# mapillary/OpenSfM

Hardware: AMD Instinct MI355X
Metric: image-pairs matched/sec (+ BA LM-iters/sec, 5k cams / 500k pts) (higher is better)
Workload: dtype i8 (exact int32 accumulate) + f64 RANSAC

## Files before the change

### opensfm_amd/csrc/ba.hip

```cpp
#ifdef OSFM_HIPEMU
#include <cassert>
#endif
#include <chrono>
#include <cmath>
#include <cstdio>
#include <cstring>
#include <numeric>
#include <vector>

#include <rocprim/rocprim.hpp>

#include "ba_math.h"
#include "osfm_internal.h"

using namespace osfm_ba;

namespace {

constexpr int kCoopObs = 256;

typedef double osfm_v2d __attribute__((ext_vector_type(2)));
__device__ __forceinline__ void st2(double *p, double a, double b) {
  osfm_v2d v;
  v.x = a;
// ... 99 lines not shown
        rho1 = a / r;
      } else {
        rho = s;
        rho1 = 1.0;
      }
      break;
    case OSFM_LOSS_CAUCHY: {
      const double sum = 1.0 + s / b;
      rho = b * log(sum);
      rho1 = 1.0 / sum;
    } break;
    default:
      rho = s;
      rho1 = 1.0;
  }
}

template <int NV, int MAXT, int N>
__device__ __forceinline__ void block_sum(double *v, double (&lds)[N]) {
  static_assert(MAXT % 64 == 0 && MAXT <= 1024, "MAXT: the kernel's launch bound, whole wavefronts");
  static_assert(N >= NV * (MAXT / 64), "block_sum: lds is shorter than NV doubles for every wavefront the launch bound allows");
#ifdef OSFM_HIPEMU
  assert((int)blockDim.x <= MAXT);
#endif
#pragma unroll
  for (int k = 0; k < NV; k++)
#pragma unroll
    for (int m = 32; m >= 1; m >>= 1) v[k] += __shfl_xor(v[k], m);
  const int lane = threadIdx.x & 63, w = threadIdx.x >> 6;
  const int nw = (blockDim.x + 63) >> 6;
  if (nw == 1) return;
  if (lane == 0)
#pragma unroll
    for (int k = 0; k < NV; k++) lds[w * NV + k] = v[k];
  __syncthreads();
  if (threadIdx.x == 0)
#pragma unroll
    for (int k = 0; k < NV; k++) {
      double s = lds[k];
      for (int w2 = 1; w2 < nw; w2++) s += lds[w2 * NV + k];
      v[k] = s;
    }
}

template <int NV, int W, int N>
__device__ __forceinline__ void shot_sum(double (&v)[NV], double (&lds)[N] ) {
  static_assert(W == 1 || N >= W * NV, "shot_sum: lds is shorter than NV doubles per wavefront");
#ifdef OSFM_HIPEMU
  assert((int)blockDim.x == 64 * W);
#endif
#pragma unroll
  for (int i = 0; i < NV; i++)
#pragma unroll
    for (int m = 32; m >= 1; m >>= 1) v[i] += __shfl_xor(v[i], m);
  if (W == 1) return;
  const int lane = threadIdx.x & 63, w = threadIdx.x >> 6;
  if (lane == 0)
#pragma unroll
    for (int i = 0; i < NV; i++) lds[w * NV + i] = v[i];
  __syncthreads();
  if (threadIdx.x == 0)
#pragma unroll
    for (int i = 0; i < NV; i++) {
      double t = lds[i];
#pragma unroll
      for (int q = 1; q < W; q++) t += lds[q * NV + i];
      v[i] = t;
    }
}
constexpr int kShotWavesSmall = 4;
constexpr int kShotWavesBelow = 1024;

__device__ __forceinline__ long xcd_contiguous(long b, long n) {
  const long q = n >> 3, r = n & 7;
  const long xcd = b & 7, within = b >> 3;
  return (xcd < r ? xcd * (q + 1) : r * (q + 1) + (xcd - r) * q) + within;
}

struct GenDev {
  int NRr;
  int KW;
  int NB;
  int NV, NRC;
  int oJp, oJc, oJb, ncomp;
  const int *view_inst, *view_rc, *view_cam;
  const int *view_col;
  const long *view_off;
  const int *inst_view0;
  const int *o_view, *sm_view;
  const unsigned char *o_kind, *sm_kind;
  double *cam, *cam_n;
  const double *cam_prior, *cam_sigma;
  double *rc, *rc_n;
  const double *rc_prior, *rc_sigma;
  double *bias, *bias_n;
  double *rcR;
  const unsigned char *rc_useful;
  const int *cam_col, *rc_col, *bias_col;
  const unsigned char *col_slot;
  double *vpart;
  double *yv;
  double *PI, *Bpri, *Cpri;
  double *gpri;
  double *bdot;
  const double *gps, *gps_sigma;
  const int *inst_bias_cam;
  const double *up, *up_sigma;
  const double *pan, *pan_sigma, *tilt, *tilt_sigma, *roll, *roll_sigma;
  const double *pt_prior, *pt_prior_sigma;
  const unsigned char *pt_prior_alt;
};

struct Dev {
  int S, P, NC;
  long M;
  int nred, cam0;
  double *cams, *poses, *pts, *cams_n, *poses_n, *pts_n;
  const double *cam_prior, *cam_sigma, *gps, *gps_sigma;
  const double *up, *up_sigma;
  double *up_r, *up_J;
  double *prior_rot;
  const uint8_t *cam_fixed, *shot_fixed, *point_fixed;
  const int *shot_camera;
  const int *cam_model;
  const double *cam_ext;
  const int *o_shot, *o_point;
  const double *o_x, *o_y, *o_sigma;
  const long *pt_off;
  const int *wg_pt;
  int nwg;
  const long *shot_off;
  const int *shot_obs;
  double *shotR;
  double *Epm;
  double *Jpm;
  double *sm_wt;
  const int *sm_shot, *sm_point;
  const double *sm_x, *sm_y, *sm_sigma;
  double *w;
  double *g_pt, *Hpp, *Hhat, *sc_pt, *D_pt, *d_pt;
  double *g_red, *diag_red, *prior_diag, *sc_red, *D_red;
  double *Hcc;
  double *Binv;
  double *part;
  double *camred;
  int bw;
  double *band;
  const unsigned char *bslot;
  double *dinv;
  const int *bp_pts;
  const int *bp_o0, *bp_last;
  const unsigned char *bp_pos;
  const int *bp_off;
  int bpNT, bpR, bpPC;
  double *bp_part;
  int cs, ncl, ncd;
  double *cD;
  double *cW, *cWt;
  double *cLi, *cLit;
  double *bD, *bE, *bG, *bH;
  double *bD2, *bGt, *bHt;
  double *bx;
  int wNB, wWb;
  double *wA, *wL, *wLt, *wDinv, *wx;
  int qcs, qm, qN;
  double *qD;
  double *qE[2];
  double *qX;
  double *qXt;
  double *qx, *qy;
  int qT;
  double *qP, *qR, *qRn, *qC;
  double *zc;
  double *y;
  double *x, *r, *z, *p, *Ap, *b;
  double *scal;
  double *partial;
  double *partial2;
  double *dotp;
  double *rrp;
  int gen;
  GenDev g;
};

#define JA(o, c) d.Jpm[(long)(c) * d.M + (o)]
constexpr int kRowComps = 17;
constexpr int R_JP = 2, R_JR = 8, R_U = 14, R_V = 15, R_WT = 16;

__device__ __forceinline__ void row_jk(const Dev &d, long o, int s, double (&jk)[6]) {
  const int ci = d.shot_camera[s];
  const double u = JA(o, R_U), v = JA(o, R_V), wt = JA(o, R_WT), sg = d.o_sigma[o];
  const double *cam = d.cams + 3 * ci;
  const double k1 = cam[0], k2 = cam[1], f = cam[2];
  const bool other = d.cam_model && d.cam_model[ci] >= 2;
  double J[6];
  jk_entries(1.0 / sg, k1, k2, f, u, v, J);
#pragma unroll
  for (int i = 0; i < 6; i++) jk[i] = other ? 0.0 : wt * J[i];
}

__global__ void shot_rot_kernel(Dev d, const double *poses) {
  const int s = blockIdx.x * blockDim.x + threadIdx.x;
  if (s >= d.S) return;
  rot_and_derivs(poses + 6 * s, d.shotR + 36 * (long)s, d.shotR + 36 * (long)s + 9);
}

struct ShotFrame {
  int model;
  const double *cam, *pose, *R;
};
__device__ __forceinline__ ShotFrame shot_frame(const Dev &d, int s) {
  const int ci = d.shot_camera[s];
  ShotFrame f;
  f.model = d.cam_model ? d.cam_model[ci] : 0;
  f.cam = f.model >= 2 ? d.cam_ext + 16 * ci : d.cams + 3 * ci;
  f.pose = d.poses + 6 * (long)s;
  f.R = d.shotR + 36 * (long)s;
  return f;
}
__device__ __forceinline__ void sm_row(const Dev &d, const ShotFrame &f, long k, double wt, double (&r)[2], double (&Jp)[6], double (&Jc)[12], double (&Jk)[6]) {
  const int p = d.sm_point[k];
  project_obs<true>(f.model, d.pts + 3 * (long)p, f.pose, f.R, f.R + 9, f.cam, d.sm_x[k], d.sm_y[k], 1.0 / d.sm_sigma[k], r, Jp, Jc, Jk);
  r[0] *= wt;
  r[1] *= wt;
#pragma unroll
  for (int i = 0; i < 6; i++) Jp[i] *= wt;
#pragma unroll
  for (int i = 0; i < 12; i++) Jc[i] *= wt;
#pragma unroll
  for (int i = 0; i < 6; i++) Jk[i] *= wt;
}

template <bool JAC>
__global__ void __launch_bounds__(kCoopObs) eval_kernel(Dev d, const double *cams, const double *poses, const double *pts, int loss, double a) {
  __shared__ double c[JAC ? 9 : 1][kCoopObs];
  __shared__ double lds[8];
  const int tid = threadIdx.x;
  const int p0 = d.wg_pt[blockIdx.x], p1 = d.wg_pt[blockIdx.x + 1];
  const long o0 = d.pt_off[p0], o1 = d.pt_off[p1];
  double acc[2] = {0.0, 0.0};
  auto compute = [&](long o, double (&row)[kRowComps]) {
    const int s = d.o_shot[o], p = d.o_point[o];
    const double *R = d.shotR + 36 * (long)s;
    double r[2], Jp[6], Jc[12], Jk[6], uv[2];
    const double sg = d.o_sigma[o];
    const int cmodel = d.cam_model ? d.cam_model[d.shot_camera[s]] : 0;
    project_obs<JAC>(cmodel, pts + 3 * (long)p, poses + 6 * (long)s, R, R + 9, cmodel >= 2 ? d.cam_ext + 16 * d.shot_camera[s] : cams + 3 * d.shot_camera[s], d.o_x[o],
                     d.o_y[o], 1.0 / sg, r, Jp, Jc, Jk, uv);
    const double sq = r[0] * r[0] + r[1] * r[1];
    double rho, rho1;
    loss_eval(loss, a, sq, rho, rho1);
    acc[0] += 0.5 * rho;
    acc[1] += sq * sg * sg;
    if (JAC) {
      const double wt = sqrt(rho1);
      row[0] = wt * r[0];
      row[1] = wt * r[1];
#pragma unroll
      for (int i = 0; i < 6; i++) row[R_JP + i] = wt * Jp[i];
#pragma unroll
      for (int i = 0; i < 2; i++)
#pragma unroll
        for (int k = 0; k < 3; k++) row[R_JR + 3 * i + k] = wt * Jc[6 * i + k];
      row[R_U] = uv[0];
      row[R_V] = uv[1];
      row[R_WT] = wt;
    }
  };
  auto products = [&](const double (&row)[kRowComps], double (&v)[9]) {
    const double r0 = row[0], r1 = row[1];
    const double *jp = row + R_JP;
#pragma unroll
    for (int j = 0; j < 3; j++) v[j] = jp[j] * r0 + jp[3 + j] * r1;
    v[3] = jp[0] * jp[0] + jp[3] * jp[3];
    v[4] = jp[0] * jp[1] + jp[3] * jp[4];
    v[5] = jp[0] * jp[2] + jp[3] * jp[5];
    v[6] = jp[1] * jp[1] + jp[4] * jp[4];
    v[7] = jp[1] * jp[2] + jp[4] * jp[5];
    v[8] = jp[2] * jp[2] + jp[5] * jp[5];
  };
  auto store = [&](long o, const double (&row)[kRowComps]) {
#pragma unroll
    for (int i = 0; i < kRowComps; i++) __builtin_nontemporal_store(row[i], &JA(o, i));
    if (d.Epm) {
      const double *jp = row + R_JP;
      double2 *dst = reinterpret_cast<double2 *>(d.Epm + 18 * o);
#pragma unroll
      for (int i = 0; i < 6; i += 2) {
        const double a0 = i < 3 ? row[R_JR + i] : -jp[i - 3], b0 = i < 3 ? row[R_JR + 3 + i] : -jp[3 + i - 3];
        const double a1 = i + 1 < 3 ? row[R_JR + i + 1] : -jp[i + 1 - 3], b1 = i + 1 < 3 ? row[R_JR + 3 + i + 1] : -jp[3 + i + 1 - 3];
        double e[6];
#pragma unroll
        for (int j = 0; j < 3; j++) {
          e[j] = a0 * jp[j] + b0 * jp[3 + j];
          e[3 + j] = a1 * jp[j] + b1 * jp[3 + j];
        }
        st2(reinterpret_cast<double *>(dst + 3 * (i / 2)), e[0], e[1]);
        st2(reinterpret_cast<double *>(dst + 3 * (i / 2) + 1), e[2], e[3]);
        st2(reinterpret_cast<double *>(dst + 3 * (i / 2) + 2), e[4], e[5]);
      }
    }
  };
  if (o1 - o0 <= kCoopObs) {
    const bool on = tid < o1 - o0;
    double row[kRowComps];
    if (on) {
      compute(o0 + tid, row);
// ... 448 lines not shown

__device__ __forceinline__ void jred_jp(const Dev &d, long k, double E[6][3]) {
  const double2 *src = reinterpret_cast<const double2 *>(d.Epm + 18 * (long)d.shot_obs[k]);
#pragma unroll
  for (int q = 0; q < 9; q++) {
    const double2 v = src[q];
    E[(2 * q) / 3][(2 * q) % 3] = v.x;
    E[(2 * q + 1) / 3][(2 * q + 1) % 3] = v.y;
  }
}
__global__ void __launch_bounds__(TPB) band_assemble_kernel(Dev d, double radius, int copies, int dk_lo, int ndk) {
  extern __shared__ __attribute__((aligned(16))) double acc[];
  const int s = (int)xcd_contiguous(blockIdx.x, gridDim.x), nb = ndk * 36;
  const int copy = threadIdx.x & (copies - 1);
  for (int t = threadIdx.x; t < nb * copies; t += TPB) acc[t] = 0.0;
  __syncthreads();
  for (long k = d.shot_off[s] + threadIdx.x; k < d.shot_off[s + 1]; k += TPB) {
    const int p = d.sm_point[k];
    const double *Hh = d.Hhat + 6 * (long)p;
    const double h[9] = {Hh[0], Hh[1], Hh[2], Hh[1], Hh[3], Hh[4], Hh[2], Hh[4], Hh[5]};
    double Ea[6][3], EH[6][3];
    jred_jp(d, k, Ea);
#pragma unroll
    for (int i = 0; i < 6; i++)
#pragma unroll
      for (int j = 0; j < 3; j++) EH[i][j] = Ea[i][0] * h[j] + Ea[i][1] * h[3 + j] + Ea[i][2] * h[6 + j];
    for (long o2 = d.pt_off[p]; o2 < d.pt_off[p + 1]; o2++) {
      const int dk = s - d.o_shot[o2] - dk_lo;
      if (dk < 0 || dk >= ndk) continue;
      double Eb[6][3];
      {
        const double2 *src = reinterpret_cast<const double2 *>(d.Epm + 18 * o2);
#pragma unroll
        for (int q = 0; q < 9; q++) {
          const double2 v = src[q];
          Eb[(2 * q) / 3][(2 * q) % 3] = v.x;
          Eb[(2 * q + 1) / 3][(2 * q + 1) % 3] = v.y;
        }
      }
#pragma unroll
      for (int i = 0; i < 6; i++)
#pragma unroll
        for (int j = 0; j < 6; j++)
          atomicAdd(&acc[(dk * 36 + i * 6 + j) * copies + copy], EH[i][0] * Eb[j][0] + EH[i][1] * Eb[j][1] + EH[i][2] * Eb[j][2]);
    }
  }
  __syncthreads();
  for (int t = threadIdx.x; t < nb; t += TPB) {
    const int dk = dk_lo + t / 36, ij = t % 36, i = ij / 6, j = ij % 6;
    const int s2 = s - dk;
    double val = 0.0;
    if (s2 >= 0) {
      double sum = 0.0;
      for (int c = 0; c < copies; c++) sum += acc[t * copies + c];
      val = -sum;
      if (dk == 0) {
        const int hi = i > j ? i : j, lo = i > j ? j : i;
        val += d.Hcc[21 * (long)s + hi * (hi + 1) / 2 + lo];
        if (i == j) val += d.prior_diag[6 * s + i];
      }
      val *= d.sc_red[6 * s + i] * d.sc_red[6 * s2 + j];
      if (dk == 0 && i == j) val += d.D_red[6 * s + i] / radius;
    }
    d.band[((long)s * (d.bw + 1) + dk) * 36 + ij] = val;
  }
}

__global__ void __launch_bounds__(TPB) band_slots_kernel(Dev d, unsigned char *table, int *max_slots) {
  extern __shared__ int bs_present[];
  const int s = blockIdx.x, R1 = d.bw + 1;
  for (int t = threadIdx.x; t < R1; t += TPB) bs_present[t] = 0;
  __syncthreads();
  for (long k = d.shot_off[s] + threadIdx.x; k < d.shot_off[s + 1]; k += TPB) {
    const int p = d.sm_point[k];
    for (long o2 = d.pt_off[p]; o2 < d.pt_off[p + 1]; o2++) {
      const int dk = s - d.o_shot[o2];
      if (dk >= 0 && dk <= d.bw) bs_present[dk] = 1;
    }
  }
  __syncthreads();
  if (threadIdx.x == 0) {
    int n = 0;
    for (int t = 0; t < R1; t++) {
      const bool on = bs_present[t] != 0 || t == 0;
      table[(long)s * R1 + t] = on ? (unsigned char)(n < 255 ? n : 255) : (unsigned char)255;
      n += on ? 1 : 0;
    }
    atomicMax(max_slots, n);
  }
}
__global__ void __launch_bounds__(TPB) band_assemble_compact_kernel(Dev d, double radius, int copies, int nslots) {
  extern __shared__ __attribute__((aligned(16))) double acc[];
  const int s = (int)xcd_contiguous(blockIdx.x, gridDim.x), R1 = d.bw + 1;
  unsigned char *slot = reinterpret_cast<unsigned char *>(acc + (long)nslots * 36 * copies);
  const int copy = threadIdx.x & (copies - 1);
  for (int t = threadIdx.x; t < nslots * 36 * copies; t += TPB) acc[t] = 0.0;
  for (int t = threadIdx.x; t < R1; t += TPB) slot[t] = d.bslot[(long)s * R1 + t];
  __syncthreads();
  for (long k = d.shot_off[s] + threadIdx.x; k < d.shot_off[s + 1]; k += TPB) {
    const int p = d.sm_point[k];
    const double *Hh = d.Hhat + 6 * (long)p;
    const double h[9] = {Hh[0], Hh[1], Hh[2], Hh[1], Hh[3], Hh[4], Hh[2], Hh[4], Hh[5]};
    double Ea[6][3], EH[6][3];
    jred_jp(d, k, Ea);
#pragma unroll
    for (int i = 0; i < 6; i++)
#pragma unroll
      for (int j = 0; j < 3; j++) EH[i][j] = Ea[i][0] * h[j] + Ea[i][1] * h[3 + j] + Ea[i][2] * h[6 + j];
    for (long o2 = d.pt_off[p]; o2 < d.pt_off[p + 1]; o2++) {
      const int dk = s - d.o_shot[o2];
      if (dk < 0 || dk > d.bw) continue;
      const int sl = slot[dk];
      double Eb[6][3];
      {
        const double2 *src = reinterpret_cast<const double2 *>(d.Epm + 18 * o2);
#pragma unroll
        for (int q = 0; q < 9; q++) {
          const double2 v = src[q];
          Eb[(2 * q) / 3][(2 * q) % 3] = v.x;
          Eb[(2 * q + 1) / 3][(2 * q + 1) % 3] = v.y;
        }
      }
#pragma unroll
      for (int i = 0; i < 6; i++)
#pragma unroll
        for (int j = 0; j < 6; j++)
          atomicAdd(&acc[(sl * 36 + i * 6 + j) * copies + copy], EH[i][0] * Eb[j][0] + EH[i][1] * Eb[j][1] + EH[i][2] * Eb[j][2]);
    }
  }
  __syncthreads();
  for (int t = threadIdx.x; t < R1 * 36; t += TPB) {
    const int dk = t / 36, ij = t % 36, i = ij / 6, j = ij % 6;
    const int s2 = s - dk, sl = slot[dk];
    double val = 0.0;
    if (s2 >= 0) {
      double sum = 0.0;
      if (sl != 255)
        for (int c = 0; c < copies; c++) sum += acc[(sl * 36 + ij) * copies + c];
      val = -sum;
      if (dk == 0) {
        const int hi = i > j ? i : j, lo = i > j ? j : i;
        val += d.Hcc[21 * (long)s + hi * (hi + 1) / 2 + lo];
        if (i == j) val += d.prior_diag[6 * s + i];
      }
      val *= d.sc_red[6 * s + i] * d.sc_red[6 * s2 + j];
      if (dk == 0 && i == j) val += d.D_red[6 * s + i] / radius;
    }
    d.band[((long)s * R1 + dk) * 36 + ij] = val;
  }
}

constexpr int kBmSlots = 128;
constexpr int kBmStride = kBmSlots + 8;
typedef double bm_v4d __attribute__((ext_vector_type(4)));

__device__ __forceinline__ void bm_lds_barrier() { asm volatile("s_waitcnt lgkmcnt(0)\n\ts_barrier" ::: "memory"); }

template <int NT>
__global__ void __launch_bounds__(384) band_mfma_kernel(Dev d) {
  constexpr int NTILES = NT * (NT + 1) / 2, MAXT = (NTILES + 3) / 4;
  constexpr int kBuf = 36 * kBmStride;
  extern __shared__ __attribute__((aligned(16))) double bm_lds[];
  const int TL = d.bw + 1, PC = d.bpPC;
  const int a = blockIdx.x / d.bpR, part = blockIdx.x - a * d.bpR;
  const int n_all = d.bp_off[a + 1] - d.bp_off[a];
  const int i0 = d.bp_off[a] + (int)((long)n_all * part / d.bpR), i1 = d.bp_off[a] + (int)((long)n_all * (part + 1) / d.bpR);
  const int nch = (i1 - i0 + PC - 1) / PC;
  const int wave = threadIdx.x >> 6, lane = threadIdx.x & 63;
  if (threadIdx.x < 72) bm_lds[(threadIdx.x / 36) * kBuf + (threadIdx.x % 36) * kBmStride + kBmSlots] = 0.0;
  if (wave >= 4) {
    const int lt = threadIdx.x - 256;
    const int ut = lt / TL, ush = lt - ut * TL;
    const bool loader = ut < PC;
    const int u = ut * TL + ush;
    int n_p, n_o0, n_k;
    auto fetch_index = [&](int c) {
      const bool on = loader && c + ut < i1;
      const long r = on ? c + ut : i0 < i1 ? i0 : 0;
      n_p = d.bp_pts[r];
      n_o0 = d.bp_o0[r];
      const int k = d.bp_pos[16 * r + ush];
      n_k = on ? k : 255;
    };
    double jv[18], hh[6];
    bool c_have = false;
    auto fetch_blocks = [&]() {
      c_have = n_k != 255;
      const long o = n_o0 + (c_have ? n_k : 0);
      const int rot1 = d.gen ? 14 : R_JR + 3, tr0 = R_JP, tr1 = R_JP + 3;
      const double sgn = -1.0;
#pragma unroll
      for (int x = 0; x < 6; x++) jv[x] = JA(o, R_JP + x);
#pragma unroll
      for (int x = 0; x < 3; x++) {
        jv[6 + x] = JA(o, R_JR + x);
        jv[12 + x] = JA(o, rot1 + x);
        jv[9 + x] = sgn * JA(o, tr0 + x);
        jv[15 + x] = sgn * JA(o, tr1 + x);
      }
      const double *Hh = d.Hhat + 6L * n_p;
#pragma unroll
      for (int x = 0; x < 6; x++) hh[x] = Hh[x];
    };
    fetch_index(i0);
    fetch_blocks();
    fetch_index(i0 + PC);
    for (int c = 0; c <= nch; c++) {
      if (c < nch && loader) {
        double *Es = bm_lds + (c & 1) * kBuf, *Fs = Es + 18 * kBmStride;
        const double zf = c_have ? 1.0 : 0.0;
        double E[18];
#pragma unroll
        for (int i = 0; i < 6; i++)
#pragma unroll
          for (int j = 0; j < 3; j++) E[3 * i + j] = jv[6 + i] * jv[j] + jv[12 + i] * jv[3 + j];
        const double h[9] = {hh[0], hh[1], hh[2], hh[1], hh[3], hh[4], hh[2], hh[4], hh[5]};
#pragma unroll
        for (int i = 0; i < 6; i++)
#pragma unroll
          for (int j = 0; j < 3; j++) {
            Es[(3 * i + j) * kBmStride + u] = c_have ? E[3 * i + j] : 0.0;
            Fs[(3 * i + j) * kBmStride + u] = zf * (E[3 * i] * h[j] + E[3 * i + 1] * h[3 + j] + E[3 * i + 2] * h[6 + j]);
          }
      }
      fetch_blocks();
      fetch_index(i0 + (c + 2) * PC);
      bm_lds_barrier();
    }
    return;
  }
  const int li = lane & 15, kk = lane >> 4;
  int adA[MAXT], adB[MAXT];
  bool have[MAXT];
#pragma unroll
  for (int m = 0; m < MAXT; m++) {
    const int tau = wave + 4 * m;
    int I = 0;
    while ((I + 1) * (I + 2) / 2 <= tau) I++;
    const int J = tau - I * (I + 1) / 2;
    have[m] = tau < NTILES;
    const int yA = 16 * I + li, yB = 16 * J + li;
    const int sA = yA / 6, sB = yB / 6;
    adA[m] = (have[m] && kk < 3 && sA <= d.bw) ? ((yA - 6 * sA) * 3 + kk) * kBmStride + sA : -1;
    adB[m] = (have[m] && kk < 3 && sB <= d.bw) ? ((yB - 6 * sB) * 3 + kk) * kBmStride + sB : -1;
  }
  bm_v4d acc[MAXT];
#pragma unroll
  for (int m = 0; m < MAXT; m++) acc[m] = (bm_v4d){0.0, 0.0, 0.0, 0.0};
  for (int c = 0; c <= nch; c++) {
    if (c >= 1) {
      const int npt = min(PC, i1 - (i0 + (c - 1) * PC));
      const int bo = ((c - 1) & 1) * kBuf;
      int ia[MAXT], ib[MAXT];
#pragma unroll
      for (int m = 0; m < MAXT; m++) {
        ia[m] = bo + 18 * kBmStride + (adA[m] < 0 ? kBmSlots : adA[m]);
        ib[m] = bo + (adB[m] < 0 ? kBmSlots : adB[m]);
      }
      for (int t = 0; t < npt; t++) {
        double va[MAXT], vb[MAXT];
#pragma unroll
        for (int m = 0; m < MAXT; m++) {
          va[m] = bm_lds[ia[m]];
          vb[m] = bm_lds[ib[m]];
          ia[m] += adA[m] < 0 ? 0 : TL;
          ib[m] += adB[m] < 0 ? 0 : TL;
        }
#pragma unroll
        for (int m = 0; m < MAXT; m++) acc[m] = __builtin_amdgcn_mfma_f64_16x16x4f64(va[m], vb[m], acc[m], 0, 0, 0);
      }
    }
    bm_lds_barrier();
  }
#pragma unroll
  for (int m = 0; m < MAXT; m++)
    if (have[m]) {
      double *dst = d.bp_part + ((long)blockIdx.x * NTILES + wave + 4 * m) * 256 + lane;
#pragma unroll
      for (int r = 0; r < 4; r++) dst[64 * r] = acc[m][r];
    }
}

__global__ void __launch_bounds__(TPB) band_finish_kernel(Dev d, double radius) {
  const long t = (long)blockIdx.x * TPB + threadIdx.x;
  const int R1 = d.bw + 1;
  if (t >= (long)d.S * R1 * 36) return;
  const int ij = (int)(t % 36), dk = (int)((t / 36) % R1), s = (int)(t / (36 * R1));
  const int i = ij / 6, j = ij - 6 * i, s2 = s - dk;
  double val = 0.0;
  if (s2 >= 0) {
    double sum = 0.0;
    const int ntiles = d.bpNT * (d.bpNT + 1) / 2;
    for (int a = max(0, s - d.bw); a <= s2; a++) {
      int row = 6 * (s - a) + i, col = 6 * (s2 - a) + j;
      if (col > row) {
        const int tmp = row;
        row = col;
        col = tmp;
      }
      const int I = row >> 4, J = col >> 4, ri = row & 15, cj = col & 15;
      const long e = ((long)(I * (I + 1) / 2 + J) * 4 + (ri >> 2)) * 64 + ((ri & 3) << 4) + cj;
      for (int r = 0; r < d.bpR; r++) sum += d.bp_part[((long)a * d.bpR + r) * ntiles * 256 + e];
    }
    val = -sum;
    if (dk == 0) {
      const int hi = i > j ? i : j, lo = i > j ? j : i;
      val += d.Hcc[21 * (long)s + hi * (hi + 1) / 2 + lo];
      if (i == j) val += d.prior_diag[6 * s + i];
    }
    val *= d.sc_red[6 * s + i] * d.sc_red[6 * s2 + j];
    if (dk == 0 && i == j) val += d.D_red[6 * s + i] / radius;
  }
  d.band[t] = val;
}

__global__ void __launch_bounds__(64) band_cholesky_kernel(Dev d, int *status) {
  extern __shared__ __attribute__((aligned(16))) double lds[];
  const int R = d.bw + 1;
  constexpr int NR = kMaxBw + 1;
  double *ring = lds;
  double *dinvr = ring + NR * R * 36;
  double *T = dinvr + NR * 36;
  double *Lc = T + 36;
  const int lane = threadIdx.x;
  const int r = lane / 6, c = lane % 6;
  int bad = 0;
  if (lane == 0) *status = 0;
  constexpr int kPre = ((kMaxBw + 1) * 36 + 63) / 64;
  double pre[kPre];
#pragma unroll
  for (int u = 0; u < kPre; u++) pre[u] = (lane + 64 * u < R * 36) ? d.band[lane + 64 * u] : 0.0;
  for (int i = 0; i < d.S; i++) {
    double *cur = ring + (i & kMaxBw) * R * 36;
#pragma unroll
    for (int u = 0; u < kPre; u++)
      if (lane + 64 * u < R * 36) cur[lane + 64 * u] = pre[u];
    if (i + 1 < d.S) {
#pragma unroll
      for (int u = 0; u < kPre; u++) pre[u] = (lane + 64 * u < R * 36) ? d.band[(long)(i + 1) * R * 36 + lane + 64 * u] : 0.0;
    }
    WAVE_SYNC();
    for (int kk = d.bw; kk >= 1; kk--) {
      const int j = i - kk;
      if (j < 0) continue;
      const double *rowj = ring + (j & kMaxBw) * R * 36;
      if (lane < 36) {
        const int m0 = (i - d.bw > j - d.bw ? i - d.bw : j - d.bw);
        double a0 = 0, a1 = 0, a2 = 0;
        for (int m = (m0 < 0 ? 0 : m0); m < j; m++) {
          const double *Lim = cur + (i - m) * 36, *Ljm = rowj + (j - m) * 36;
          a0 += Lim[r * 6 + 0] * Ljm[c * 6 + 0] + Lim[r * 6 + 3] * Ljm[c * 6 + 3];
          a1 += Lim[r * 6 + 1] * Ljm[c * 6 + 1] + Lim[r * 6 + 4] * Ljm[c * 6 + 4];
          a2 += Lim[r * 6 + 2] * Ljm[c * 6 + 2] + Lim[r * 6 + 5] * Ljm[c * 6 + 5];
        }
        T[lane] = cur[kk * 36 + lane] - ((a0 + a1) + a2);
      }
      WAVE_SYNC();
      if (lane < 36) {
        const double *dj = dinvr + (j & kMaxBw) * 36;
        double v = 0;
#pragma unroll
        for (int q = 0; q < 6; q++) v += T[r * 6 + q] * dj[c * 6 + q];
        cur[kk * 36 + lane] = v;
      }
      WAVE_SYNC();
    }
    if (lane < 36) {
      const int m0 = i - d.bw;
      double a0 = 0, a1 = 0, a2 = 0;
      for (int m = (m0 < 0 ? 0 : m0); m < i; m++) {
        const double *Lim = cur + (i - m) * 36;
        a0 += Lim[r * 6 + 0] * Lim[c * 6 + 0] + Lim[r * 6 + 3] * Lim[c * 6 + 3];
        a1 += Lim[r * 6 + 1] * Lim[c * 6 + 1] + Lim[r * 6 + 4] * Lim[c * 6 + 4];
        a2 += Lim[r * 6 + 2] * Lim[c * 6 + 2] + Lim[r * 6 + 5] * Lim[c * 6 + 5];
      }
      T[lane] = cur[lane] - ((a0 + a1) + a2);
      Lc[lane] = 0.0;
    }
    WAVE_SYNC();
    for (int cc = 0; cc < 6; cc++) {
      if (lane < 6 && lane >= cc) {
        double sum = T[lane * 6 + cc];
        for (int q = 0; q < cc; q++) sum -= Lc[lane * 6 + q] * Lc[cc * 6 + q];
        if (lane == cc) {
          if (!(sum > 0)) { bad = 1; sum = 1.0; }
          Lc[cc * 6 + cc] = sqrt(sum);
        } else {
          T[lane * 6 + cc] = sum;
        }
      }
      WAVE_SYNC();
      if (lane < 6 && lane > cc) Lc[lane * 6 + cc] = T[lane * 6 + cc] / Lc[cc * 6 + cc];
      WAVE_SYNC();
    }
    double *di = dinvr + (i & kMaxBw) * 36;
    if (lane < 6) {
      const int cc = lane;
      double col[6];
      for (int rr = 0; rr < 6; rr++) {
        double sum = (rr == cc) ? 1.0 : 0.0;
        for (int q = cc; q < rr; q++) sum -= Lc[rr * 6 + q] * col[q];
        col[rr] = (rr >= cc) ? sum / Lc[rr * 6 + rr] : 0.0;
      }
      for (int rr = 0; rr < 6; rr++) di[rr * 6 + cc] = col[rr];
    }
    if (lane < 36) cur[lane] = Lc[lane];
    WAVE_SYNC();
    for (int t = lane; t < R * 36; t += 64) d.band[(long)i * R * 36 + t] = cur[t];
    if (lane < 36) d.dinv[(long)i * 36 + lane] = di[lane];
    WAVE_SYNC();
  }
  if (bad) *status = 1;
}

constexpr int kPD = 4;
template <int BW>
__global__ void __launch_bounds__(64) band_solve_kernel(Dev d, const double *rin, double *z) {
  __shared__ double part[36];
  __shared__ double tv[6];
  __shared__ double yring[(kMaxBw + 1) * 6];
  constexpr int R = BW + 1;
  constexpr long kRow = (long)R * 36;
  const int lane = threadIdx.x, r = lane / 6, c = lane % 6;
  const int l36 = lane < 36 ? lane : 0, l6 = lane < 6 ? lane : 0;
  const int lt = lane < 36 ? c * 6 + r : 0;
  double pb[kPD][BW], pdv[kPD][6], pr[kPD];
  for (int t = lane; t < (kMaxBw + 1) * 6; t += 64) yring[t] = 0.0;
  WAVE_SYNC();
  const double *bp = d.band + 36 + l36;
  const double *dp = d.dinv + l6 * 6;
#pragma unroll
  for (int u = 0; u < kPD; u++) {
    const long row = u < d.S ? u : d.S - 1;
// ... 4015 lines not shown
    (void)rocprim::radix_sort_pairs(nullptr, need3, first_shot, bp_keys, iota, bp_pts, (size_t)NP, 0u, fbits, sv.st);
    const size_t tb = std::max(std::max(need1, need2), need3);
    unsigned char *tmp = A.alloc<unsigned char>(tb + 256, e);
    OSFM_REQUIRE(e == hipSuccess, OSFM_E_NOMEM, "BA device allocation/upload failed: %s", hipGetErrorString(e));
    hipLaunchKernelGGL(iota_int_kernel, dim3(nblk(M)), dim3(TPB), 0, sv.st, iota, M);
    size_t tb1 = tb, tb2 = tb;
    OSFM_HIP(rocprim::radix_sort_pairs(tmp, tb1, raw_point, o_point, iota, d_perm, (size_t)M, 0u, pbits, sv.st));
    hipLaunchKernelGGL(gather_int_kernel, dim3(nblk(M)), dim3(TPB), 0, sv.st, d_perm, raw_shot, M, o_shot);
    hipLaunchKernelGGL(lower_bound_kernel, dim3(nblk(NP + 1L)), dim3(TPB), 0, sv.st, o_point, M, NP, d_pt_off);
    if (gen) {
      hipLaunchKernelGGL(gather_int_kernel, dim3(nblk(M)), dim3(TPB), 0, sv.st, d_perm, raw_view, M, o_view);
      OSFM_HIP(rocprim::radix_sort_pairs(tmp, tb2, o_view, sm_keys, iota, shot_obs, (size_t)M, 0u, sbits, sv.st));
      hipLaunchKernelGGL(lower_bound_kernel, dim3(nblk(g.NV + 1L)), dim3(TPB), 0, sv.st, sm_keys, M, g.NV, d_view_off);
      hipLaunchKernelGGL(gen_shot_off_kernel, dim3(nblk(S + 1L)), dim3(TPB), 0, sv.st, (const long *)d_view_off, g.inst_view0, S, d_shot_off);
      g.o_view = o_view;
      g.sm_view = sm_keys;
      g.view_off = d_view_off;
    } else {
      OSFM_HIP(rocprim::radix_sort_pairs(tmp, tb2, o_shot, sm_keys, iota, shot_obs, (size_t)M, 0u, sbits, sv.st));
      hipLaunchKernelGGL(lower_bound_kernel, dim3(nblk(S + 1L)), dim3(TPB), 0, sv.st, sm_keys, M, S, d_shot_off);
    }
    OSFM_HIP(hipMemsetAsync(d_bw, 0, 2 * sizeof(int), sv.st));
    hipLaunchKernelGGL(track_width_kernel, dim3(nblk(NP)), dim3(TPB), 0, sv.st, d_pt_off, o_shot, NP, d_bw);
    hipLaunchKernelGGL(track_first_kernel, dim3(nblk(NP)), dim3(TPB), 0, sv.st, d_pt_off, o_shot, NP, S, first_shot, d_bw + 1);
    if ((long)NP <= M) {
      size_t tb3 = tb;
      OSFM_HIP(rocprim::radix_sort_pairs(tmp, tb3, first_shot, bp_keys, iota, bp_pts, (size_t)NP, 0u, fbits, sv.st));
    } else
      bp_pts = nullptr;
    OSFM_HIP(hipGetLastError());
    OSFM_HIP(hipMemcpyAsync(pt_off.data(), d_pt_off, ((size_t)NP + 1) * sizeof(long), hipMemcpyDeviceToHost, sv.st));
    OSFM_HIP(hipMemcpyAsync(&pl.bw_true, d_bw, sizeof(int), hipMemcpyDeviceToHost, sv.st));
    OSFM_HIP(hipMemcpyAsync(&pl.track_repeats_shot, d_bw + 1, sizeof(int), hipMemcpyDeviceToHost, sv.st));
    OSFM_HIP(hipStreamSynchronize(sv.st));
    d.o_shot = o_shot;
    d.o_point = o_point;
    d.pt_off = d_pt_off;
    d.shot_off = d_shot_off;
    d.shot_obs = shot_obs;
  }
  {
    double *raw_xy = A.upload(P->obs_xy, (size_t)2 * M, e), *raw_sg = A.upload(P->obs_sigma, (size_t)M, e);
    double *ox = A.alloc<double>((size_t)M, e), *oy = A.alloc<double>((size_t)M, e), *osg = A.alloc<double>((size_t)M, e);
    if (e == hipSuccess && M > 0) hipLaunchKernelGGL(gather_pm_kernel, dim3(nblk(M)), dim3(TPB), 0, sv.st, d_perm, raw_xy, raw_sg, M, ox, oy, osg);
    d.o_x = ox;
    d.o_y = oy;
    d.o_sigma = osg;
    if (gen && G->obs_kind && M > 0) {
      unsigned char *raw_kind = A.upload(G->obs_kind, (size_t)M, e), *ok = A.alloc<unsigned char>((size_t)M, e), *sk = A.alloc<unsigned char>((size_t)M, e);
      if (e == hipSuccess) {
        hipLaunchKernelGGL(gather_byte_kernel, dim3(nblk(M)), dim3(TPB), 0, sv.st, (const int *)d_perm, (const unsigned char *)raw_kind, M, ok);
        hipLaunchKernelGGL(gather_byte_kernel, dim3(nblk(M)), dim3(TPB), 0, sv.st, d.shot_obs, (const unsigned char *)ok, M, sk);
      }
      g.o_kind = ok;
      g.sm_kind = sk;
    }
  }
  {
    std::vector<int> wg_pt;
    wg_pt.push_back(0);
    int pcur = 0;
    while (pcur < NP) {
      int pe = pcur + 1;
      while (pe < NP && pe - pcur < kCoopObs && pt_off[(size_t)pe + 1] - pt_off[(size_t)pcur] <= kCoopObs) pe++;
      wg_pt.push_back(pe);
      pcur = pe;
    }
    if (wg_pt.size() < 2) wg_pt.push_back(0);
    d.nwg = (int)wg_pt.size() - 1;
    d.wg_pt = A.upload(wg_pt.data(), wg_pt.size(), e);
  }
  pl.bp_keys = bp_keys;
  pl.bp_pts = bp_pts;
  return OSFM_OK;
}

static void alloc_work_vectors(Arena &A, hipError_t &e, Solver &sv, int nbord) {
  Dev &d = sv.d;
  GenDev &g = d.g;
  const bool gen = d.gen != 0;
  const int S = d.S, NP = d.P, NC = d.NC;
  const long M = d.M;
  d.shotR = A.alloc<double>((size_t)36 * S, e);
  d.Jpm = A.alloc<double>((size_t)(gen ? g.ncomp : kRowComps) * M, e);
  d.sm_wt = A.alloc<double>((size_t)std::max<long>(1, M), e);
  {
    int *ss = A.alloc<int>((size_t)M, e), *sp = A.alloc<int>((size_t)M, e);
    double *sx = A.alloc<double>((size_t)M, e), *sy = A.alloc<double>((size_t)M, e), *ssg = A.alloc<double>((size_t)M, e);
    if (e == hipSuccess && M > 0)
      hipLaunchKernelGGL(gather_sm_kernel, dim3(nblk(M)), dim3(TPB), 0, sv.st, d.shot_obs, d.o_shot, d.o_point, d.o_x, d.o_y, d.o_sigma, M, ss,
                         sp, sx, sy, ssg);
    d.sm_shot = ss;
    d.sm_point = sp;
    d.sm_x = sx;
    d.sm_y = sy;
    d.sm_sigma = ssg;
  }
  d.w = A.alloc<double>((size_t)(gen ? g.NRr : 2) * M, e);
  d.g_pt = A.alloc<double>((size_t)3 * NP, e);
  d.Hpp = A.alloc<double>((size_t)6 * NP, e);
  d.Hhat = A.alloc<double>((size_t)6 * NP, e);
  d.sc_pt = A.alloc<double>((size_t)3 * NP, e);
  d.D_pt = A.alloc<double>((size_t)3 * NP, e);
  d.d_pt = A.alloc<double>((size_t)3 * NP, e);
  const size_t nr = (size_t)d.nred;
  d.g_red = A.alloc<double>(nr, e);
  d.diag_red = A.alloc<double>(nr, e);
  d.prior_diag = A.alloc<double>(nr, e);
  d.sc_red = A.alloc<double>(nr, e);
  d.D_red = A.alloc<double>(nr, e);
  d.Hcc = A.alloc<double>((size_t)21 * S + 6 * NC, e);
  d.Binv = A.alloc<double>((size_t)36 * S + 9 * NC + nbord, e);
  d.part = A.alloc<double>((size_t)9 * S, e);
  d.camred = A.alloc<double>((size_t)9 * NC, e);
  d.zc = A.alloc<double>(nr, e);
  d.y = A.alloc<double>(nr, e);
  d.x = A.alloc<double>(nr, e);
  d.r = A.alloc<double>(nr, e);
  d.z = A.alloc<double>(nr, e);
  d.p = A.alloc<double>(nr, e);
  d.Ap = A.alloc<double>(nr, e);
  d.b = A.alloc<double>(nr, e);
  d.scal = A.alloc<double>(32, e);
  const long nbmax = std::max<long>(std::max<long>(nblk(M), nblk(3L * NP)), d.nwg);
  d.partial = A.alloc<double>((size_t)2 * nbmax + 16, e);
  d.partial2 = A.alloc<double>((size_t)2 * nblk(3L * NP) + 16, e);
  d.dotp = A.alloc<double>((size_t)nblk(d.nred) + NC + 16, e);
  d.rrp = A.alloc<double>((size_t)nblk(d.nred) + 16, e);
}

static int choose_band_solver(osfm_ctx *ctx, const osfm_ba_options *O, Arena &A, hipError_t &e, Solver &sv, SolvePlan &pl) {
  Dev &d = sv.d;
  GenDev &g = d.g;
  const BaSwitches &sw = sv.sw;
  const bool gen = d.gen != 0;
  const int S = d.S, NP = d.P;
  const long M = d.M;
  constexpr int kLdsBw = 10;
  static_assert(kLdsBw <= kSbMaxBw, "the one-workgroup band factor runs on the LDS clusters' bands");
  pl.wide = O->preconditioner == 0 && S >= 2 && pl.bw_true > kLdsBw && pl.bw_true <= kWMaxBw;
  d.bw = O->preconditioner == 1 ? 0 : (pl.wide ? pl.bw_true : std::min(pl.bw_true, kMaxBw));
  if (S < 2) d.bw = 0;
  const int band_nslice = (d.bw + 1 + kBandSlice - 1) / kBandSlice;
  pl.band_slice = (d.bw + 1 + band_nslice - 1) / band_nslice;
  pl.band_copies = kBandCopies;
  while (pl.band_copies > 1 && (size_t)pl.band_slice * 36 * pl.band_copies * sizeof(double) > 150 * 1024) pl.band_copies /= 2;
  d.band = A.alloc<double>((size_t)S * (d.bw + 1) * 36, e);
  pl.win_band = d.bw >= 1 && d.bw <= kMaxBw && d.bw == pl.bw_true && !pl.track_repeats_shot && pl.bp_pts != nullptr && !sw.band_per_shot &&
                !(gen && g.NRr == 3);
  d.Epm = d.bw > 0 && (!pl.win_band || sw.check_band) ? A.alloc<double>((size_t)18 * M, e) : nullptr;
  if (pl.win_band) {
    const int TL = d.bw + 1;
    d.bpNT = (6 * TL + 15) / 16;
    d.bpPC = kBmSlots / TL;
    d.bpR = (int)std::min<long>(8, std::max<long>(1, ((long)NP + 128L * S - 1) / (128L * S)));
    pl.win_grid = S * d.bpR;
    pl.win_lds = (size_t)2 * 36 * kBmStride * sizeof(double);
    int *off = A.alloc<int>((size_t)S + 1, e), *o0 = A.alloc<int>((size_t)NP, e), *ln = A.alloc<int>((size_t)NP, e);
    unsigned char *tpos = A.alloc<unsigned char>((size_t)16 * NP, e);
    d.bp_part = A.alloc<double>((size_t)pl.win_grid * (d.bpNT * (d.bpNT + 1) / 2) * 256, e);
    d.bp_pts = pl.bp_pts;
    d.bp_off = off;
    d.bp_o0 = o0;
    d.bp_last = ln;
    d.bp_pos = tpos;
    if (e == hipSuccess) {
      hipLaunchKernelGGL(slab_bound_kernel, dim3(nblk(S + 1L)), dim3(TPB), 0, sv.st, pl.bp_keys, NP, 1, S, off);
      hipLaunchKernelGGL(sorted_tracks_kernel, dim3(nblk(NP)), dim3(TPB), 0, sv.st, pl.bp_pts, pl.bp_keys, d.pt_off, d.o_shot, NP, o0, ln, tpos);
    }
  }
  d.bslot = nullptr;
  if (d.bw > kMaxBw && !pl.win_band) {
    unsigned char *tab = A.alloc<unsigned char>((size_t)S * (d.bw + 1), e);
    int *d_mx = A.alloc<int>(1, e);
    OSFM_REQUIRE(e == hipSuccess, OSFM_E_NOMEM, "BA device allocation/upload failed: %s", hipGetErrorString(e));
    OSFM_HIP(hipMemsetAsync(d_mx, 0, sizeof(int), sv.st));
    hipLaunchKernelGGL(band_slots_kernel, dim3(S), dim3(TPB), (size_t)(d.bw + 1) * sizeof(int), sv.st, d, tab, d_mx);
    OSFM_HIP(hipMemcpyAsync(&pl.bslot_n, d_mx, sizeof(int), hipMemcpyDeviceToHost, sv.st));
    OSFM_HIP(hipStreamSynchronize(sv.st));
    if (pl.bslot_n >= 1 && pl.bslot_n <= 64) {
      d.bslot = tab;
      pl.bslot_copies = kBandCopies;
      while (pl.bslot_copies > 1 && (size_t)pl.bslot_n * 36 * pl.bslot_copies * sizeof(double) + d.bw + 1 > 72 * 1024) pl.bslot_copies /= 2;
    }
  }
  d.dinv = A.alloc<double>((size_t)S * 36, e);
  d.cs = 0; d.ncl = 0; d.ncd = 0;
  if (d.bw >= 1 && d.bw <= kLdsBw && d.bw == pl.bw_true && O->preconditioner == 0) {
    d.cs = d.bw < 2 ? 2 : d.bw;
    d.ncd = 6 * d.cs;
    d.ncl = (S + d.cs - 1) / d.cs;
    const size_t nb = (size_t)d.ncl * d.ncd * d.ncd;
    d.cD = A.alloc<double>(nb, e);
    d.cW = A.alloc<double>(nb + (size_t)d.ncd * d.ncd, e);
    d.cWt = A.alloc<double>(nb + (size_t)d.ncd * d.ncd, e);
    d.cLi = A.alloc<double>(nb, e);
    d.cLit = A.alloc<double>(nb, e);
    d.bD = A.alloc<double>(nb, e);
    d.bE = A.alloc<double>(nb, e);
    d.bG = A.alloc<double>(nb, e);
    d.bH = A.alloc<double>(nb, e);
    d.bD2 = A.alloc<double>(nb, e);
    d.bGt = A.alloc<double>(nb, e);
    d.bHt = A.alloc<double>(nb, e);
    d.bx = A.alloc<double>((size_t)kWalkRhs * d.ncl * d.ncd, e);
    sv.use_sband = d.bw <= kSbMaxBw && sband_factor_lds(S, d.bw) <= kSbLdsMax && sband_solve_lds(S, d.bw) <= kSbLdsMax && !sw.no_sband;
    if (sv.use_sband) sv.sbL = A.alloc<double>((size_t)S * (d.bw + 1) * 36, e);
  }
  d.wNB = 0; d.wWb = 0;
  d.qN = 0; d.qm = 0; d.qcs = 0;
  pl.dense_cr = pl.wide && !sw.wide_ldlt;
  if (pl.dense_cr) {
    const size_t qm = (size_t)6 * d.bw, nq = (size_t)(S + d.bw - 1) / d.bw, np = (qm + kWB - 1) / kWB, qT = ((qm + np - 1) / np + 5) / 6 * 6;
    const size_t need = (nq * qm * qm * 9 + nq * qm * 8 + (nq / 2 + 1) * (3 * qT * qT + 3 * qT * qm)) * sizeof(double);
    size_t free_b = 0, total_b = 0;
    if (sw.dense_cr_budget) free_b = (size_t)atoll(sw.dense_cr_budget);
    else if (hipMemGetInfo(&free_b, &total_b) != hipSuccess) free_b = ~(size_t)0;
    else free_b += ctx->pool_bytes;
    if (need > free_b - free_b / 8) pl.dense_cr = false;
  }
  if (pl.dense_cr) {
    d.qcs = d.bw;
    d.qm = 6 * d.qcs;
    d.qN = (S + d.qcs - 1) / d.qcs;
    const size_t m2 = (size_t)d.qm * d.qm, nq = (size_t)d.qN;
    d.qD = A.alloc<double>(nq * m2, e);
    d.qE[0] = A.alloc<double>(nq * m2, e);
    d.qE[1] = A.alloc<double>(nq * m2, e);
    d.qX = A.alloc<double>(nq * 2 * m2, e);
    d.qXt = A.alloc<double>(nq * 2 * m2, e);
    d.qx = A.alloc<double>(nq * d.qm * 4, e);
    d.qy = A.alloc<double>(nq * d.qm * 4, e);
    {
      const int np = (d.qm + kWB - 1) / kWB;
      d.qT = ((d.qm + np - 1) / np + 5) / 6 * 6;
      const size_t nb = nq / 2 + 1;
      d.qP = A.alloc<double>(nb * d.qT * d.qT, e);
      d.qR = A.alloc<double>(nb * d.qT * d.qm, e);
      d.qRn = A.alloc<double>(nb * d.qT * d.qm, e);
      d.qC = A.alloc<double>(nb * d.qT * d.qm, e);
    }
  }
  if (pl.wide && !pl.dense_cr) {
    d.wNB = (S + kWcs - 1) / kWcs;
    d.wWb = std::min((d.bw + kWcs - 1) / kWcs, d.wNB - 1);
    const size_t nt = (size_t)d.wNB * (d.wWb + 1) * kWB * kWB;
    d.wA = A.alloc<double>(nt, e);
    d.wL = A.alloc<double>(nt, e);
    d.wLt = A.alloc<double>(nt, e);
    d.wDinv = A.alloc<double>((size_t)d.wNB * kWB * kWB, e);
    d.wx = A.alloc<double>((size_t)d.wNB * kWB * 4, e);
  }
  return OSFM_OK;
}

static int plan_border_and_iteration(const osfm_ba_problem *P, const osfm_ba_options *O, const GenInput *G, Arena &A, hipError_t &e, Solver &sv, SolvePlan &pl) {
  Dev &d = sv.d;
  GenDev &g = d.g;
  const bool gen = G != nullptr;
  const int S = d.S, NC = d.NC;
  const long M = d.M;
  const int nbord = pl.nbord;
  if ((d.ncl > 0 || pl.wide) && nbord >= 1 && nbord <= (gen ? kGenMaxNB : 6)) {
    sv.Bc = A.alloc<double>((size_t)nbord * 6 * S, e);
    sv.Wb = A.alloc<double>((size_t)nbord * 6 * S, e);
    sv.SigInv = A.alloc<double>((size_t)nbord * nbord, e);
    sv.yb = A.alloc<double>((size_t)nbord + 8, e);
    sv.dots = A.alloc<double>((size_t)nbord * nbord, e);
    sv.dCm = A.alloc<double>((size_t)nbord * nbord, e);
    if (!gen) {
      sv.wB = A.alloc<double>((size_t)2 * 3 * NC * M, e);
      sv.partB = A.alloc<double>((size_t)S * 9 * NC, e);
    } else {
      std::vector<int> cols, col_pos((size_t)nbord, -1);
      for (int j = 0; j < nbord; j++) {
        bool held = false;
        for (int v = 0; v < G->NV && !held; v++) held = sv.gen_col_slot[(size_t)j * G->NV + v] != 255;
        if (held) {
          col_pos[(size_t)j] = (int)cols.size();
          cols.push_back(j);
        }
      }
      sv.g_ncols = (int)cols.size();
      if (cols.empty()) cols.push_back(0);
      sv.g_cols = A.upload(cols.data(), cols.size(), e);
      sv.g_col_pos = A.upload(col_pos.data(), col_pos.size(), e);
      sv.g_wB = A.alloc<double>((size_t)std::max<long>(1, M) * std::max(1, sv.g_ncols) * g.NRr, e);
      sv.g_vpartB = A.alloc<double>((size_t)std::max(1, G->NV) * std::max(1, sv.g_ncols) * std::max(1, g.KW), e);
    }
  }
  pl.all_cams_fixed = !gen;
  for (int c = 0; c < NC && !gen; c++) {
    if (P->cam_fixed[c]) pl.border_ok = false;
    else pl.all_cams_fixed = false;
  }
  sv.cams_inert = pl.all_cams_fixed;
  if (pl.all_cams_fixed && e == hipSuccess) OSFM_HIP(hipMemsetAsync(d.camred, 0, (size_t)9 * NC * sizeof(double), sv.st));
  pl.try_bcr = d.bw > 0 && d.ncl > 0 && O->preconditioner == 0;
  pl.try_border = (pl.try_bcr || pl.wide) && sv.Bc && pl.border_ok;
  pl.want_border = d.bw > 0 && (d.ncl > 0 || pl.wide) && O->preconditioner == 0 && sv.Bc && pl.border_ok;
  pl.sband_fuse = sv.use_sband && !gen && pl.all_cams_fixed && d.bw > 0 && d.ncl > 0 && O->preconditioner == 0 && !pl.want_border;
  pl.side2 = pl.sband_fuse ? nullptr : sv.st2;
  pl.fork_at = pl.sband_fuse ? 0 : pl.win_band ? (d.ncl > 1 && O->preconditioner == 0 ? 2 : 1) : 0;
  pl.fork_in_bcr = pl.fork_at == 2 && pl.side2 && d.bw > 0 && d.ncl > 1 && O->preconditioner == 0;
  pl.exact_expected = (pl.try_bcr || pl.wide) && (pl.try_border || (gen ? g.NB == 0 : pl.all_cams_fixed)) && O->pcg_direct_tolerance > O->pcg_tolerance;
  return OSFM_OK;
}

static int write_outputs(osfm_ba_problem *P, const GenInput *G, Arena &A, hipError_t &e, Solver &sv) {
  Dev &d = sv.d;
// ... 117 lines not shown
```

Before: 2.700 million.

## Pack four points per MFMA k-step in band Schur MFMA kernel

The band Schur-complement MFMA kernel previously issued one 16x16x4 f64 MFMA per point with only 3 of 4 k-lanes active (one lane group zero). It now lays out points at a compile-time pitch so each MFMA consumes 4 (point, component) pairs across 3 MFMAs per group of 4 points, uses full k-depth, distributes tiles contiguously per wave via templated per-wave specialisations, and software-pipelines LDS loads with double-buffered registers. This reduces MFMA count and LDS traffic per point, at the cost of a fixed pitch derived from NT that may waste slots, and more register usage per wave.

```diff
diff --git a/opensfm_amd/csrc/ba.hip b/opensfm_amd/csrc/ba.hip
--- a/opensfm_amd/csrc/ba.hip
+++ b/opensfm_amd/csrc/ba.hip
@@ -275,7 +275,7 @@
   const int *bp_o0, *bp_last;
   const unsigned char *bp_pos;
   const int *bp_off;
-  int bpNT, bpR, bpPC;
+  int bpNT, bpR;
   double *bp_part;
   int cs, ncl, ncd;
   double *cD;
@@ -1030,27 +1030,116 @@
 
 constexpr int kBmSlots = 128;
 constexpr int kBmStride = kBmSlots + 8;
+constexpr int kBmBuf = 36 * kBmStride;
+constexpr int kBmZero = 2 * kBmBuf;
+constexpr int kBmLdsBytes = (2 * kBmBuf + kBmStride) * (int)sizeof(double);
+constexpr int bm_pitch(int nt) { return 16 * nt / 6; }
+constexpr int bm_points(int nt) { return (kBmSlots / bm_pitch(nt)) & ~3; }
+constexpr int bm_tile_row(int tau) {
+  int I = 0;
+  while ((I + 1) * (I + 2) / 2 <= tau) I++;
+  return I;
+}
 typedef double bm_v4d __attribute__((ext_vector_type(4)));
 
 __device__ __forceinline__ void bm_lds_barrier() { asm volatile("s_waitcnt lgkmcnt(0)\n\ts_barrier" ::: "memory"); }
+
+__device__ __forceinline__ int bm_wave_uniform(int v) {
+#if defined(__HIP_DEVICE_COMPILE__)
+  return __builtin_amdgcn_readfirstlane(v);
+#else
+  return v;
+#endif
+}
+
+template <int NT, int W>
+__device__ __forceinline__ void bm_multiply(const Dev &d, double *bm_lds, int i0, int i1, int nch, int lane) {
+  constexpr int NTILES = NT * (NT + 1) / 2, P = bm_pitch(NT), PC = bm_points(NT), G = PC / 4;
+  constexpr int TAU0 = W * NTILES / 4, NTW = (W + 1) * NTILES / 4 - TAU0;
+  constexpr int NI = NTW * G, NA = NTW > 0 ? NTW : 1;
+  static_assert((G - 1) * 4 * P + 3 * P < kBmStride, "band_mfma_kernel: a chunk stays inside a row");
+  const int li = lane & 15, kk = lane >> 4;
+  int adA[NA][3], adB[NA][3];
+  bool inA[NA], inB[NA];
+#pragma unroll
+  for (int m = 0; m < NA; m++) {
+    const int I = bm_tile_row(TAU0 + m), J = TAU0 + m - I * (I + 1) / 2;
+    const int yA = 16 * I + li, yB = 16 * J + li;
+    const int sA = yA / 6, sB = yB / 6;
+    inA[m] = sA <= d.bw;
+    inB[m] = sB <= d.bw;
+#pragma unroll
+    for (int g = 0; g < 3; g++) {
+      const int k = 4 * g + kk, dt = k / 3, comp = k - 3 * dt;
+      adA[m][g] = inA[m] ? (18 + (yA - 6 * sA) * 3 + comp) * kBmStride + sA + dt * P : kBmZero;
+      adB[m][g] = inB[m] ? ((yB - 6 * sB) * 3 + comp) * kBmStride + sB + dt * P : kBmZero;
+    }
+  }
+  bm_v4d acc[NA];
+#pragma unroll
+  for (int m = 0; m < NA; m++) acc[m] = (bm_v4d){0.0, 0.0, 0.0, 0.0};
+  for (int c = 0; c <= nch; c++) {
+    if (c >= 1) {
+      const int npt = min(PC, i1 - (i0 + (c - 1) * PC));
+      const int ngr = (npt + 3) >> 2;
+      const int bo = ((c - 1) & 1) * kBmBuf;
+      int ia[NA][3], ib[NA][3];
+#pragma unroll
+      for (int m = 0; m < NA; m++)
+#pragma unroll
+        for (int g = 0; g < 3; g++) {
+          ia[m][g] = adA[m][g] + (inA[m] ? bo : 0);
+          ib[m][g] = adB[m][g] + (inB[m] ? bo : 0);
+        }
+      double va[2][3], vb[2][3];
+#pragma unroll
+      for (int g = 0; g < (NI > 0 ? 3 : 0); g++) {
+        va[0][g] = bm_lds[ia[0][g]];
+        vb[0][g] = bm_lds[ib[0][g]];
+      }
+#pragma unroll
+      for (int j = 0; j < NI; j++) {
+        const int m = j / G, n = j % G;
+        if (j + 1 < NI) {
+          const int m1 = (j + 1) / G, n1 = (j + 1) % G;
+#pragma unroll
+          for (int g = 0; g < 3; g++) {
+            va[(j + 1) & 1][g] = bm_lds[ia[m1][g] + n1 * 4 * P];
+            vb[(j + 1) & 1][g] = bm_lds[ib[m1][g] + n1 * 4 * P];
+          }
+        }
+        if (n < ngr) {
+#pragma unroll
+          for (int g = 0; g < 3; g++) acc[m] = __builtin_amdgcn_mfma_f64_16x16x4f64(va[j & 1][g], vb[j & 1][g], acc[m], 0, 0, 0);
+        }
+      }
+    }
+    bm_lds_barrier();
+  }
+#pragma unroll
+  for (int m = 0; m < NTW; m++) {
+    double *dst = d.bp_part + ((long)blockIdx.x * NTILES + TAU0 + m) * 256 + lane;
+#pragma unroll
+    for (int r = 0; r < 4; r++) dst[64 * r] = acc[m][r];
+  }
+}
 
 template <int NT>
 __global__ void __launch_bounds__(384) band_mfma_kernel(Dev d) {
-  constexpr int NTILES = NT * (NT + 1) / 2, MAXT = (NTILES + 3) / 4;
-  constexpr int kBuf = 36 * kBmStride;
+  constexpr int P = bm_pitch(NT), PC = bm_points(NT);
   extern __shared__ __attribute__((aligned(16))) double bm_lds[];
-  const int TL = d.bw + 1, PC = d.bpPC;
+  const int TL = d.bw + 1;
   const int a = blockIdx.x / d.bpR, part = blockIdx.x - a * d.bpR;
   const int n_all = d.bp_off[a + 1] - d.bp_off[a];
   const int i0 = d.bp_off[a] + (int)((long)n_all * part / d.bpR), i1 = d.bp_off[a] + (int)((long)n_all * (part + 1) / d.bpR);
   const int nch = (i1 - i0 + PC - 1) / PC;
-  const int wave = threadIdx.x >> 6, lane = threadIdx.x & 63;
-  if (threadIdx.x < 72) bm_lds[(threadIdx.x / 36) * kBuf + (threadIdx.x % 36) * kBmStride + kBmSlots] = 0.0;
+  const int wave = bm_wave_uniform(threadIdx.x >> 6), lane = threadIdx.x & 63;
+  if (threadIdx.x < kBmStride) bm_lds[kBmZero + threadIdx.x] = 0.0;
   if (wave >= 4) {
     const int lt = threadIdx.x - 256;
     const int ut = lt / TL, ush = lt - ut * TL;
     const bool loader = ut < PC;
-    const int u = ut * TL + ush;
+    const int u = ut * P + ush;
     int n_p, n_o0, n_k;
     auto fetch_index = [&](int c) {
       const bool on = loader && c + ut < i1;
@@ -1085,7 +1174,7 @@
     fetch_index(i0 + PC);
     for (int c = 0; c <= nch; c++) {
       if (c < nch && loader) {
-        double *Es = bm_lds + (c & 1) * kBuf, *Fs = Es + 18 * kBmStride;
+        double *Es = bm_lds + (c & 1) * kBmBuf, *Fs = Es + 18 * kBmStride;
         const double zf = c_have ? 1.0 : 0.0;
         double E[18];
 #pragma unroll
@@ -1107,56 +1196,12 @@
     }
     return;
   }
-  const int li = lane & 15, kk = lane >> 4;
-  int adA[MAXT], adB[MAXT];
-  bool have[MAXT];
-#pragma unroll
-  for (int m = 0; m < MAXT; m++) {
-    const int tau = wave + 4 * m;
-    int I = 0;
-    while ((I + 1) * (I + 2) / 2 <= tau) I++;
-    const int J = tau - I * (I + 1) / 2;
-    have[m] = tau < NTILES;
-    const int yA = 16 * I + li, yB = 16 * J + li;
-    const int sA = yA / 6, sB = yB / 6;
-    adA[m] = (have[m] && kk < 3 && sA <= d.bw) ? ((yA - 6 * sA) * 3 + kk) * kBmStride + sA : -1;
-    adB[m] = (have[m] && kk < 3 && sB <= d.bw) ? ((yB - 6 * sB) * 3 + kk) * kBmStride + sB : -1;
-  }
-  bm_v4d acc[MAXT];
-#pragma unroll
-  for (int m = 0; m < MAXT; m++) acc[m] = (bm_v4d){0.0, 0.0, 0.0, 0.0};
-  for (int c = 0; c <= nch; c++) {
-    if (c >= 1) {
-      const int npt = min(PC, i1 - (i0 + (c - 1) * PC));
-      const int bo = ((c - 1) & 1) * kBuf;
-      int ia[MAXT], ib[MAXT];
-#pragma unroll
-      for (int m = 0; m < MAXT; m++) {
-        ia[m] = bo + 18 * kBmStride + (adA[m] < 0 ? kBmSlots : adA[m]);
-        ib[m] = bo + (adB[m] < 0 ? kBmSlots : adB[m]);
-      }
-      for (int t = 0; t < npt; t++) {
-        double va[MAXT], vb[MAXT];
-#pragma unroll
-        for (int m = 0; m < MAXT; m++) {
-          va[m] = bm_lds[ia[m]];
-          vb[m] = bm_lds[ib[m]];
-          ia[m] += adA[m] < 0 ? 0 : TL;
-          ib[m] += adB[m] < 0 ? 0 : TL;
-        }
-#pragma unroll
-        for (int m = 0; m < MAXT; m++) acc[m] = __builtin_amdgcn_mfma_f64_16x16x4f64(va[m], vb[m], acc[m], 0, 0, 0);
-      }
-    }
-    bm_lds_barrier();
-  }
-#pragma unroll
-  for (int m = 0; m < MAXT; m++)
-    if (have[m]) {
-      double *dst = d.bp_part + ((long)blockIdx.x * NTILES + wave + 4 * m) * 256 + lane;
-#pragma unroll
-      for (int r = 0; r < 4; r++) dst[64 * r] = acc[m][r];
-    }
+  switch (wave) {
+    case 0: bm_multiply<NT, 0>(d, bm_lds, i0, i1, nch, lane); break;
+    case 1: bm_multiply<NT, 1>(d, bm_lds, i0, i1, nch, lane); break;
+    case 2: bm_multiply<NT, 2>(d, bm_lds, i0, i1, nch, lane); break;
+    default: bm_multiply<NT, 3>(d, bm_lds, i0, i1, nch, lane); break;
+  }
 }
 
 __global__ void __launch_bounds__(TPB) band_finish_kernel(Dev d, double radius) {
@@ -5478,10 +5523,9 @@
   if (pl.win_band) {
     const int TL = d.bw + 1;
     d.bpNT = (6 * TL + 15) / 16;
-    d.bpPC = kBmSlots / TL;
     d.bpR = (int)std::min<long>(8, std::max<long>(1, ((long)NP + 128L * S - 1) / (128L * S)));
     pl.win_grid = S * d.bpR;
-    pl.win_lds = (size_t)2 * 36 * kBmStride * sizeof(double);
+    pl.win_lds = kBmLdsBytes;
     int *off = A.alloc<int>((size_t)S + 1, e), *o0 = A.alloc<int>((size_t)NP, e), *ln = A.alloc<int>((size_t)NP, e);
     unsigned char *tpos = A.alloc<unsigned char>((size_t)16 * NP, e);
     d.bp_part = A.alloc<double>((size_t)pl.win_grid * (d.bpNT * (d.bpNT + 1) / 2) * 256, e);
```

Result: no change. 2.693 million (-0.3%).
